# matthiasverstraete/3d_recognizer

Measured on AMD Instinct MI355X. Metric: training clouds/sec, N=40960 pts, bs=8, at 1/2/4/8 GPUs; mIoU parity, higher is better.
Workload: dtype f32 storage/accumulate, bf16x3 MFMA in the wide GEMMs

## Files before the change

3d_recognizer_amd/csrc/knn_grid.hip:

```cpp
#include "rl_common.h"
#include <stdlib.h>

namespace {

constexpr int KNN_SB = 3;


struct GridGeom {
    float lo[3];
    float inv[3];
    float h[3];
    int n[3];
    int ncell;
    float slack;
};

__device__ __forceinline__ unsigned enc(float f) {
    const unsigned u = __float_as_uint(f);
    return (u & 0x80000000u) ? ~u : (u | 0x80000000u);
}
__device__ __forceinline__ float dec(unsigned u) {
    return __uint_as_float((u & 0x80000000u) ? (u & 0x7fffffffu) : ~u);
}

constexpr int KNN_MAX_TASKS = 8;

struct KTask {
    const float* S;
    long s_bs;
    const float* Q;
    long q_bs;
    int Ns, Nq, k, self_mode;
    int32_t* idx32;
    int64_t* idx64;
    float* d2;
    GridGeom* geom;
    unsigned* bbox;
    int* count;
    int* start;
    int* cursor;
    float4* sorted;
    int cstride, maxcells;
    float per_cell;
    int lanes;
};

struct KMulti {
    int ntasks, B;
    int xcd;
    KTask t[KNN_MAX_TASKS];
};

__device__ __forceinline__ void knn_deal(const KMulti& m, int& b, int& bx) {
    if (m.xcd) {
        const int lin = (int)blockIdx.x + (int)gridDim.x * b;
        b = lin % m.B;
        bx = lin / m.B;
    }
}

__device__ __forceinline__ int kmax_of(int k) { return k == 1 ? 1 : k <= 4 ? 4 : k <= 8 ? 8 : k <= 16 ? 16 : k <= 32 ? 32 : 64; }

__global__ __launch_bounds__(256) void grid_init_kernel(const KMulti m) {
    const int task = blockIdx.y / m.B, b = blockIdx.y % m.B;
    const KTask& T = m.t[task];
    const int i = blockIdx.x * 256 + threadIdx.x;
    if (i < 6) T.bbox[b * 6 + i] = (i < 3) ? 0xffffffffu : 0u;
    int* cnt = T.count + (size_t)b * T.cstride;
    for (int e = i; e < T.cstride; e += gridDim.x * 256) cnt[e] = 0;
}

__global__ __launch_bounds__(256) void grid_bbox_kernel(const KMulti m) {
    const int task = blockIdx.y / m.B, b = blockIdx.y % m.B;
    const KTask& T = m.t[task];
    if (blockIdx.x * 256 >= T.Ns) return;
    const float* Sb = T.S + (size_t)b * T.s_bs * 3;
    float mn[3] = {INFINITY, INFINITY, INFINITY}, mx[3] = {-INFINITY, -INFINITY, -INFINITY};
    for (int j = blockIdx.x * 256 + threadIdx.x; j < T.Ns; j += gridDim.x * 256) {
#pragma unroll
        for (int a = 0; a < 3; ++a) {
            const float v = Sb[(size_t)j * 3 + a];
            mn[a] = fminf(mn[a], v);
            mx[a] = fmaxf(mx[a], v);
        }
    }
#pragma unroll
    for (int a = 0; a < 3; ++a) {
#pragma unroll
        for (int o = 32; o > 0; o >>= 1) {
            mn[a] = fminf(mn[a], __shfl_xor(mn[a], o, 64));
            mx[a] = fmaxf(mx[a], __shfl_xor(mx[a], o, 64));
        }
    }
    __shared__ float red[4][6];
    if ((threadIdx.x & 63) == 0) {
#pragma unroll
        for (int a = 0; a < 3; ++a) {
// ... 138 lines not shown
    }
}

template <int KMAX, int SB>
__device__ __forceinline__ void take_batch(const float4 (&cand)[SB], unsigned valid, float qx, float qy, float qz,
                                           unsigned long long (&best)[KMAX]) {
    unsigned long long key[SB];
    unsigned pass = 0;
#pragma unroll
    for (int i = 0; i < SB; ++i) {
        const float4 c = cand[i];
        const float dx = __fsub_rn(qx, c.x), dy = __fsub_rn(qy, c.y), dz = __fsub_rn(qz, c.z);
        const float d = __fadd_rn(__fadd_rn(__fmul_rn(dx, dx), __fmul_rn(dy, dy)), __fmul_rn(dz, dz));
        key[i] = ((unsigned long long)__float_as_uint(d) << 32) | (unsigned)__float_as_int(c.w);
        if (((valid >> i) & 1u) && key[i] < best[KMAX - 1]) pass |= 1u << i;
    }
    while (pass) {
        const int i = __ffs(pass) - 1;
        pass &= pass - 1;
        unsigned long long kk = key[0];
#pragma unroll
        for (int j = 1; j < SB; ++j)
            if (j == i) kk = key[j];
        insert_key<KMAX>(kk, best);
    }
}

template <int KMAX>
__device__ __forceinline__ void scan_range(const float4* __restrict__ pts, int begin, int end, float qx, float qy,
                                           float qz, unsigned long long (&best)[KMAX]) {
    constexpr int SB = KNN_SB;
    for (int t = begin; t < end; t += SB) {
        float4 cand[SB];
        unsigned valid = 0;
#pragma unroll
        for (int i = 0; i < SB; ++i) {
            cand[i] = pts[min(t + i, end - 1)];
            if (t + i < end) valid |= 1u << i;
        }
        take_batch<KMAX, SB>(cand, valid, qx, qy, qz, best);
    }
}

__device__ __forceinline__ int centre_out(int t) { return (t & 1) ? -((t + 1) >> 1) : (t >> 1); }

__device__ __forceinline__ float axis_gap(const GridGeom& g, int a, int ci, float q) {
    const float lo = g.lo[a] + (float)ci * g.h[a];
    const float hi = lo + g.h[a];
    float gap = fmaxf(lo - q, q - hi);
    gap -= g.slack;
    return gap > 0.f ? gap : 0.f;
}

template <int KMAX>
__device__ __forceinline__ void query_one_lane(const KTask& T, int b, int bx) {
    const int k = T.k, Nq = T.Nq, Ns = T.Ns;
    const int t = bx * 256 + threadIdx.x;
    if (t >= Nq) return;
    const int self_mode = T.self_mode;
    const float* Q = T.Q;
    const long q_bs = T.q_bs;
    int32_t* idx32 = T.idx32;
    int64_t* idx64 = T.idx64;
    float* d2out = T.d2;
    const GridGeom g = T.geom[b];
    const float4* pts = T.sorted + (size_t)b * Ns;
    const int* st = T.start + (size_t)b * T.cstride;
    float qx, qy, qz;
    int qi;
    if (self_mode) {
        const float4 me = pts[t];
        qx = me.x; qy = me.y; qz = me.z;
        qi = __float_as_int(me.w);
    } else {
        const float* p = Q + ((size_t)b * q_bs + t) * 3;
        qx = p[0]; qy = p[1]; qz = p[2];
        qi = t;
    }
    int c[3];
    cell_coords(g, qx, qy, qz, c);
    unsigned long long best[KMAX];
#pragma unroll
    for (int s = 0; s < KMAX; ++s) best[s] = KEY_EMPTY;

    const float q3[3] = {qx, qy, qz};
    for (int r = 0;; ++r) {
        const int z0 = max(c[2] - r, 0), z1 = min(c[2] + r, g.n[2] - 1);
        const int y0 = max(c[1] - r, 0), y1 = min(c[1] + r, g.n[1] - 1);
        const int x0 = max(c[0] - r, 0), x1 = min(c[0] + r, g.n[0] - 1);
        for (int tz = 0; tz <= 2 * r; ++tz) {
            const int z = c[2] + centre_out(tz);
            if (z < z0 || z > z1) continue;
            const bool zedge = (z == c[2] - r) || (z == c[2] + r);
            const float dz = axis_gap(g, 2, z, qz);
            for (int ty = 0; ty <= 2 * r; ++ty) {
                const int y = c[1] + centre_out(ty);
                if (y < y0 || y > y1) continue;
                const bool full_row = zedge || y == c[1] - r || y == c[1] + r;
                const float dy = axis_gap(g, 1, y, qy);
                const float dyz = dy * dy + dz * dz;
                const int row = (z * g.n[1] + y) * g.n[0];
                unsigned long long kth = best[KMAX - 1];
                if (k != KMAX) {
#pragma unroll
                    for (int s = 0; s < KMAX; ++s)
                        if (s == k - 1) kth = best[s];
                }
                const bool have = kth != KEY_EMPTY;
                const float lim = have ? __uint_as_float((unsigned)(kth >> 32)) * 1.00001f + 1e-30f : INFINITY;
                if (dyz > lim) continue;
                if (full_row) {
                    int xa = x0, xb = x1;
                    while (xa <= xb) {
                        const float gx = axis_gap(g, 0, xa, qx);
                        if (gx * gx + dyz > lim) ++xa; else break;
                    }
                    while (xb >= xa) {
                        const float gx = axis_gap(g, 0, xb, qx);
                        if (gx * gx + dyz > lim) --xb; else break;
                    }
                    if (xa <= xb) scan_range<KMAX>(pts, st[row + xa], st[row + xb + 1], qx, qy, qz, best);
                } else {
#pragma unroll
                    for (int e = 0; e < 2; ++e) {
                        const int x = e == 0 ? c[0] - r : c[0] + r;
                        if (x < x0 || x > x1 || (e == 1 && r == 0)) continue;
                        const float dxg = axis_gap(g, 0, x, qx);
                        if (dxg * dxg + dyz > lim) continue;
                        scan_range<KMAX>(pts, st[row + x], st[row + x + 1], qx, qy, qz, best);
                    }
                }
            }
        }
        const bool covers = (c[0] - r <= 0) && (c[0] + r >= g.n[0] - 1) && (c[1] - r <= 0) && (c[1] + r >= g.n[1] - 1) &&
                            (c[2] - r <= 0) && (c[2] + r >= g.n[2] - 1);
        if (covers) break;
        unsigned long long kth = best[KMAX - 1];
#pragma unroll
        for (int s = 0; s < KMAX; ++s)
            if (s == k - 1) kth = best[s];
        if (kth != KEY_EMPTY) {
            float bound = INFINITY;
#pragma unroll
            for (int a = 0; a < 3; ++a) {
                if (c[a] - r > 0) bound = fminf(bound, q3[a] - (g.lo[a] + (float)(c[a] - r) * g.h[a]));
                if (c[a] + r < g.n[a] - 1) bound = fminf(bound, (g.lo[a] + (float)(c[a] + r + 1) * g.h[a]) - q3[a]);
            }
            bound -= g.slack;
            const float kd = __uint_as_float((unsigned)(kth >> 32));
            if (bound > 0.f && kd < bound * bound * 0.999999f) break;
        }
    }
    const size_t o = ((size_t)b * Nq + qi) * k;
#pragma unroll
    for (int s = 0; s < KMAX; ++s) {
        if (s < k) {
            const bool empty = best[s] == KEY_EMPTY;
            const unsigned id = empty ? 0xffffffffu : (unsigned)(best[s] & 0xffffffffull);
            if (idx32) idx32[o + s] = (int32_t)id;
            if (idx64) idx64[o + s] = (int64_t)id;
            d2out[o + s] = __uint_as_float(empty ? 0xffffffffu : (unsigned)(best[s] >> 32));
        }
    }
}

template <int LANES>
__device__ __forceinline__ unsigned long long group_min(unsigned long long v) {
#pragma unroll
    for (int o = 1; o < LANES; o <<= 1) {
        const unsigned lo = __shfl_xor((unsigned)v, o, 64), hi = __shfl_xor((unsigned)(v >> 32), o, 64);
        const unsigned long long w = ((unsigned long long)hi << 32) | lo;
        v = w < v ? w : v;
    }
    return v;
}
template <int LANES>
__device__ __forceinline__ unsigned long long group_max(unsigned long long v) {
#pragma unroll
    for (int o = 1; o < LANES; o <<= 1) {
        const unsigned lo = __shfl_xor((unsigned)v, o, 64), hi = __shfl_xor((unsigned)(v >> 32), o, 64);
        const unsigned long long w = ((unsigned long long)hi << 32) | lo;
        v = w > v ? w : v;
    }
    return v;
}

template <int KMAX, int LANES>
__device__ __forceinline__ unsigned long long group_bound(const unsigned long long (&best)[KMAX], int k) {
    const int q = (k + LANES - 1) / LANES - 1;
    unsigned long long own_k = best[KMAX - 1], own_q = best[0];
#pragma unroll
    for (int s = 0; s < KMAX; ++s) {
        if (s == k - 1) own_k = best[s];
        if (s == q) own_q = best[s];
    }
    const unsigned long long a = group_min<LANES>(own_k), b = group_max<LANES>(own_q);
    return a < b ? a : b;
}

template <int KMAX, int LANES>
__device__ __forceinline__ void scan_range_n(const float4* __restrict__ pts, int begin, int end, int sub, float qx, float qy,
                                            float qz, unsigned long long (&best)[KMAX]) {
    constexpr int SB = KNN_SB;
    for (int t = begin + sub; t < end; t += LANES * SB) {
        float4 cand[SB];
        unsigned valid = 0;
#pragma unroll
        for (int i = 0; i < SB; ++i) {
            cand[i] = pts[min(t + LANES * i, end - 1)];
            if (t + LANES * i < end) valid |= 1u << i;
        }
        take_batch<KMAX, SB>(cand, valid, qx, qy, qz, best);
    }
}

template <int KMAX, int LANES>
__device__ __forceinline__ void query_n_lanes(const KTask& T, int b, int bx, unsigned long long* lds) {
    constexpr int QPB = 256 / LANES;
    unsigned long long (*lists)[LANES][KMAX] = reinterpret_cast<unsigned long long (*)[LANES][KMAX]>(lds);
    const int k = T.k, Nq = T.Nq, Ns = T.Ns;
    const int qslot = threadIdx.x / LANES, sub = threadIdx.x % LANES;
    const int t = bx * QPB + qslot;
    if (bx * QPB >= Nq) return;
    const bool active = t < Nq;
    unsigned long long best[KMAX];
#pragma unroll
    for (int s = 0; s < KMAX; ++s) best[s] = KEY_EMPTY;
    int qi = 0;
    if (active) {
        const GridGeom g = T.geom[b];
        const float4* pts = T.sorted + (size_t)b * Ns;
        const int* st = T.start + (size_t)b * T.cstride;
        float qx, qy, qz;
        if (T.self_mode) {
            const float4 me = pts[t];
            qx = me.x; qy = me.y; qz = me.z;
            qi = __float_as_int(me.w);
        } else {
            const float* p = T.Q + ((size_t)b * T.q_bs + t) * 3;
            qx = p[0]; qy = p[1]; qz = p[2];
            qi = t;
        }
        int c[3];
        cell_coords(g, qx, qy, qz, c);
        const float q3[3] = {qx, qy, qz};
        for (int r = 0;; ++r) {
            const int z0 = max(c[2] - r, 0), z1 = min(c[2] + r, g.n[2] - 1);
            const int y0 = max(c[1] - r, 0), y1 = min(c[1] + r, g.n[1] - 1);
            const int x0 = max(c[0] - r, 0), x1 = min(c[0] + r, g.n[0] - 1);
            for (int tz = 0; tz <= 2 * r; ++tz) {
                const int z = c[2] + centre_out(tz);
                if (z < z0 || z > z1) continue;
                const bool zedge = (z == c[2] - r) || (z == c[2] + r);
                const float dz = axis_gap(g, 2, z, qz);
                for (int ty = 0; ty <= 2 * r; ++ty) {
                    const int y = c[1] + centre_out(ty);
                    if (y < y0 || y > y1) continue;
                    const bool full_row = zedge || y == c[1] - r || y == c[1] + r;
                    const float dy = axis_gap(g, 1, y, qy);
                    const float dyz = dy * dy + dz * dz;
                    const int row = (z * g.n[1] + y) * g.n[0];
                    const unsigned long long kth = group_bound<KMAX, LANES>(best, k);
                    const float lim = kth != KEY_EMPTY ? __uint_as_float((unsigned)(kth >> 32)) * 1.00001f + 1e-30f : INFINITY;
                    if (dyz > lim) continue;
                    if (full_row) {
                        int xa = x0, xb = x1;
                        while (xa <= xb) {
                            const float gx = axis_gap(g, 0, xa, qx);
                            if (gx * gx + dyz > lim) ++xa; else break;
                        }
                        while (xb >= xa) {
                            const float gx = axis_gap(g, 0, xb, qx);
                            if (gx * gx + dyz > lim) --xb; else break;
                        }
                        if (xa <= xb) scan_range_n<KMAX, LANES>(pts, st[row + xa], st[row + xb + 1], sub, qx, qy, qz, best);
                    } else {
#pragma unroll
                        for (int e = 0; e < 2; ++e) {
                            const int x = e == 0 ? c[0] - r : c[0] + r;
                            if (x < x0 || x > x1 || (e == 1 && r == 0)) continue;
                            const float dxg = axis_gap(g, 0, x, qx);
                            if (dxg * dxg + dyz > lim) continue;
                            scan_range_n<KMAX, LANES>(pts, st[row + x], st[row + x + 1], sub, qx, qy, qz, best);
                        }
                    }
                }
            }
            const bool covers = (c[0] - r <= 0) && (c[0] + r >= g.n[0] - 1) && (c[1] - r <= 0) && (c[1] + r >= g.n[1] - 1) &&
                                (c[2] - r <= 0) && (c[2] + r >= g.n[2] - 1);
            if (covers) break;
            const unsigned long long kth = group_bound<KMAX, LANES>(best, k);
            if (kth != KEY_EMPTY) {
                float bound = INFINITY;
#pragma unroll
                for (int a = 0; a < 3; ++a) {
                    if (c[a] - r > 0) bound = fminf(bound, q3[a] - (g.lo[a] + (float)(c[a] - r) * g.h[a]));
                    if (c[a] + r < g.n[a] - 1) bound = fminf(bound, (g.lo[a] + (float)(c[a] + r + 1) * g.h[a]) - q3[a]);
                }
                bound -= g.slack;
                const float kd = __uint_as_float((unsigned)(kth >> 32));
                if (bound > 0.f && kd < bound * bound * 0.999999f) break;
            }
        }
    }
#pragma unroll
    for (int s = 0; s < KMAX; ++s) lists[qslot][sub][s] = best[s];
    __syncthreads();
    if (active) {
        const size_t o = ((size_t)b * Nq + qi) * k;
#pragma unroll
        for (int s = 0; s < KMAX; ++s) {
            const unsigned long long key = best[s];
            if (key == KEY_EMPTY) continue;
            int rank = s;
#pragma unroll
            for (int j = 1; j < LANES; ++j) {
                const unsigned long long* L = lists[qslot][(sub + j) % LANES];
                int lo = 0;
#pragma unroll
                for (int w = KMAX / 2; w >= 1; w >>= 1)
                    if (L[lo + w - 1] < key) lo += w;
                if (lo < KMAX && L[lo] < key) ++lo;
                rank += lo;
            }
            if (rank < k) {
                const unsigned id = (unsigned)(key & 0xffffffffull);
                if (T.idx32) T.idx32[o + rank] = (int32_t)id;
                if (T.idx64) T.idx64[o + rank] = (int64_t)id;
                T.d2[o + rank] = __uint_as_float((unsigned)(key >> 32));
            }
        }
    }
}

template <int KMAX>
__global__ __launch_bounds__(256, KMAX <= 16 ? 4 : 1) void grid_query_kernel(const KMulti m) {
    __shared__ unsigned long long lds[KMAX <= 16 ? 256 * KMAX : 1];
    const int task = blockIdx.y / m.B;
    int b = blockIdx.y % m.B, bx = blockIdx.x;
    knn_deal(m, b, bx);
    const KTask& T = m.t[task];
    if (kmax_of(T.k) != KMAX) return;
    if constexpr (KMAX <= 16) {
        if (T.lanes == 4) { query_n_lanes<KMAX, 4>(T, b, bx, lds); return; }
        if (T.lanes == 2) { query_n_lanes<KMAX, 2>(T, b, bx, lds); return; }
    }
    query_one_lane<KMAX>(T, b, bx);
}

struct Plan {
    int maxcells, cstride;
    float per_cell;
    size_t off_geom, off_bbox, off_count, off_start, off_cursor, off_sorted, bytes;
};

Plan make_plan(int B, int Ns, int k) {
    Plan p;
    constexpr float occ = 0.5f;
    p.per_cell = fmaxf(2.f, occ * (float)k);
    const long want = (long)((double)Ns / p.per_cell) + 1;
    p.maxcells = (int)(4 * want + 64);
    p.cstride = p.maxcells + 1;
    size_t o = 0;
    auto take = [&](size_t n) { size_t at = o; o += (n + 255) & ~(size_t)255; return at; };
    p.off_geom = take(sizeof(GridGeom) * B);
    p.off_bbox = take(sizeof(unsigned) * 6 * B);
    p.off_count = take(sizeof(int) * (size_t)p.cstride * B);
    p.off_start = take(sizeof(int) * (size_t)p.cstride * B);
    p.off_cursor = take(sizeof(int) * (size_t)p.cstride * B);
    p.off_sorted = take(sizeof(float4) * (size_t)Ns * B);
    p.bytes = o;
    return p;
}

void bind(KTask* t, const Plan& p, char* w) {
    t->geom = (GridGeom*)(w + p.off_geom);
    t->bbox = (unsigned*)(w + p.off_bbox);
    t->count = (int*)(w + p.off_count);
    t->start = (int*)(w + p.off_start);
    t->cursor = (int*)(w + p.off_cursor);
    t->sorted = (float4*)(w + p.off_sorted);
    t->cstride = p.cstride;
    t->maxcells = p.maxcells;
    t->per_cell = p.per_cell;
}

inline int lanes_for(long queries, int k) {
    if (k > 16) return 1;
    return queries >= 16384 ? 1 : 4;
}

int run_multi(const KMulti& m_in, hipStream_t st) {
    KMulti m = m_in;
    m.xcd = (m.B > 1 && 8 % m.B == 0) ? 1 : 0;
    for (int i = 0; i < m.ntasks; ++i) m.t[i].lanes = lanes_for((long)m.B * m.t[i].Nq, m.t[i].k);
    int maxNs = 1, maxNq = 1, maxc = 1;
    bool need[6] = {false, false, false, false, false, false};
    for (int i = 0; i < m.ntasks; ++i) {
        maxNs = max(maxNs, m.t[i].Ns);
        maxNq = max(maxNq, m.t[i].Nq);
        maxc = max(maxc, m.t[i].cstride);
        const int k = m.t[i].k;
        need[k == 1 ? 0 : k <= 4 ? 1 : k <= 8 ? 2 : k <= 16 ? 3 : k <= 32 ? 4 : 5] = true;
    }
    const int clouds = m.ntasks * m.B;
    int gi = rl_cdiv(maxc, 256);
    if (gi > 64) gi = 64;
    hipLaunchKernelGGL(grid_init_kernel, dim3(gi, clouds), dim3(256), 0, st, m);
    int gb = rl_cdiv(maxNs, 2048);
    if (gb > 16) gb = 16;
    hipLaunchKernelGGL(grid_bbox_kernel, dim3(gb, clouds), dim3(256), 0, st, m);
    hipLaunchKernelGGL(grid_geom_kernel, dim3(rl_cdiv(clouds, 64)), dim3(64), 0, st, m);
    hipLaunchKernelGGL(grid_count_kernel, dim3(rl_cdiv(maxNs, 256), clouds), dim3(256), 0, st, m);
    hipLaunchKernelGGL(grid_scan_kernel, dim3(clouds), dim3(1024), 0, st, m);
    hipLaunchKernelGGL(grid_scatter_kernel, dim3(rl_cdiv(maxNs, 256), clouds), dim3(256), 0, st, m);
    int gxq = 1;
    for (int i = 0; i < m.ntasks; ++i) gxq = max(gxq, rl_cdiv((long)m.t[i].Nq * m.t[i].lanes, 256));
    dim3 grid(gxq, clouds);
    if (need[0]) hipLaunchKernelGGL((grid_query_kernel<1>), grid, dim3(256), 0, st, m);
    if (need[1]) hipLaunchKernelGGL((grid_query_kernel<4>), grid, dim3(256), 0, st, m);
    if (need[2]) hipLaunchKernelGGL((grid_query_kernel<8>), grid, dim3(256), 0, st, m);
    if (need[3]) hipLaunchKernelGGL((grid_query_kernel<16>), grid, dim3(256), 0, st, m);
    if (need[4]) hipLaunchKernelGGL((grid_query_kernel<32>), grid, dim3(256), 0, st, m);
    if (need[5]) hipLaunchKernelGGL((grid_query_kernel<64>), grid, dim3(256), 0, st, m);
    rl_note_kernel("grid_query_kernel");
    RL_LAUNCH_CHECK("rl_knn(grid)");
    return RL_OK;
}

}

int64_t rl_knn_grid_workspace_bytes(int B, int Ns, int k) { return (int64_t)make_plan(B, Ns, k).bytes; }

int rl_knn_grid_run(const float* S, long s_bs, const float* Q, long q_bs, int B, int Ns, int Nq, int k, int32_t* i32,
                    int64_t* i64, float* d2, void* workspace, int64_t workspace_bytes, hipStream_t st) {
    const Plan p = make_plan(B, Ns, k);
    RL_REQUIRE(workspace && workspace_bytes >= (int64_t)p.bytes, RL_ERR_ARGS, "rl_knn: workspace too small (%ld < %ld bytes)",
               (long)workspace_bytes, (long)p.bytes);
    RL_REQUIRE(((uintptr_t)workspace & 255) == 0, RL_ERR_ARGS, "rl_knn: workspace must be 256-byte aligned");
    KMulti m;
    m.ntasks = 1;
    m.B = B;
    KTask& t = m.t[0];
    t.S = S; t.s_bs = s_bs; t.Q = Q; t.q_bs = q_bs; t.Ns = Ns; t.Nq = Nq; t.k = k;
    t.self_mode = (S == Q && s_bs == q_bs && Ns == Nq) ? 1 : 0;
    t.idx32 = i32; t.idx64 = i64; t.d2 = d2;
    bind(&t, p, (char*)workspace);
    return run_multi(m, st);
}

extern "C" int64_t rl_knn_multi_workspace_bytes(const rl_knn_task* tasks, int ntasks, int B) {
    if (!tasks || ntasks <= 0 || B <= 0) return 0;
    int64_t total = 0;
    for (int i = 0; i < ntasks; ++i) total += (int64_t)make_plan(B, tasks[i].Ns, tasks[i].k).bytes;
    return total;
}

extern "C" int rl_knn_multi(const rl_knn_task* tasks, int ntasks, int B, void* workspace, int64_t workspace_bytes,
                            void* stream) {
    RL_REQUIRE(tasks && ntasks > 0 && ntasks <= KNN_MAX_TASKS && B > 0 && B * ntasks <= 65535, RL_ERR_ARGS,
               "rl_knn_multi: 1..%d tasks expected", KNN_MAX_TASKS);
    RL_REQUIRE(workspace && ((uintptr_t)workspace & 255) == 0, RL_ERR_ARGS, "rl_knn_multi: workspace must be 256-byte aligned");
    KMulti m;
    m.ntasks = ntasks;
    m.B = B;
    size_t off = 0;
    for (int i = 0; i < ntasks; ++i) {
        const rl_knn_task& u = tasks[i];
        RL_REQUIRE(u.support && u.query && u.idx_out && u.d2_out && u.Nq > 0 && u.k > 0, RL_ERR_ARGS, "rl_knn_multi: bad task %d", i);
        RL_REQUIRE(u.Ns >= u.k, RL_ERR_FEW_SUPPORT, "Not enough points in support to find %d neighboors", u.k);
        RL_REQUIRE(u.k <= RL_KNN_MAX_K, RL_ERR_UNSUPPORTED, "rl_knn_multi: k=%d exceeds RL_KNN_MAX_K=%d", u.k, RL_KNN_MAX_K);
        RL_REQUIRE(u.support_bstride >= u.Ns && u.query_bstride >= u.Nq, RL_ERR_ARGS, "rl_knn_multi: batch stride smaller than the cloud");
        const Plan p = make_plan(B, u.Ns, u.k);
        RL_REQUIRE((int64_t)(off + p.bytes) <= workspace_bytes, RL_ERR_ARGS, "rl_knn_multi: workspace too small");
        KTask& t = m.t[i];
        t.S = u.support; t.s_bs = u.support_bstride; t.Q = u.query; t.q_bs = u.query_bstride;
        t.Ns = u.Ns; t.Nq = u.Nq; t.k = u.k;
        t.self_mode = (u.support == u.query && u.support_bstride == u.query_bstride && u.Ns == u.Nq) ? 1 : 0;
        t.idx32 = u.idx_out; t.idx64 = nullptr; t.d2 = u.d2_out;
        bind(&t, p, (char*)workspace + off);
        off += p.bytes;
    }
    return run_multi(m, (hipStream_t)stream);
// ... 2 lines not shown
```

3d_recognizer_amd/randlanet/_hip.py:

```python
import ctypes as C
import os
from typing import Optional

import torch

_LIB: Optional[C.CDLL] = None
_LIB_PATH = os.path.join(os.path.dirname(os.path.dirname(os.path.abspath(__file__))), "csrc",
                         "librandla_hip.so")
_LIB_PATH = os.environ.get("RL_HIP_LIB", _LIB_PATH)

ABI_VERSION = 110
MAX_SLOTS = 1024
KNN_MAX_K = 64
ACT_NONE, ACT_RELU, ACT_LRELU = 0, 1, 2

ERR_ARGS, ERR_FEW_SUPPORT, ERR_LAUNCH, ERR_UNSUPPORTED = -1, -2, -3, -4


class HipKernelError(RuntimeError):
    pass


class GemmDesc(C.Structure):
    _fields_ = [
# ... 219 lines not shown
    "rl_wgrad_plan": (_i, [C.POINTER(WgradDesc), C.POINTER(C.c_int32), C.POINTER(C.c_int32), C.POINTER(C.c_char_p)]),
    "rl_wgrad_plan2": (_i, [C.POINTER(WgradDesc), C.POINTER(C.c_int32), C.POINTER(C.c_int32), C.POINTER(C.c_char_p),
                            C.POINTER(C.c_int32), C.POINTER(C.c_int64), C.POINTER(C.c_int32), C.POINTER(C.c_char_p)]),
    "rl_gemm_plan": (_i, [C.POINTER(GemmDesc), C.POINTER(C.c_int32), C.POINTER(C.c_int32), C.POINTER(C.c_int32), C.POINTER(C.c_int32),
                          C.POINTER(C.c_int32), C.POINTER(C.c_char_p), C.POINTER(C.c_char_p)]),
    "rl_wgrad_nsplit": (_i, [_l, _i, _i]),
    "rl_wgrad_batchable": (_i, [C.POINTER(WgradDesc)]),
    "rl_wgrad_batch": (_i, [C.POINTER(WgradDesc), _i, _vp]),
    "rl_wgrad_reduce_batch": (_i, [C.POINTER(WgradReduceItem), _i, _vp]),
    "rl_bn_finalize": (_i, [_vp, _i, _l, _i, _vp, _vp, _vp, _vp, _vp, _f, _f, _i, _vp, _vp, _vp, _vp, _vp, _i, _vp, _vp]),
    "rl_bn_finalize_batch": (_i, [C.POINTER(BnFinalizeItem), _i, _vp]),
    "rl_bn_bwd_finalize_batch": (_i, [C.POINTER(BnBwdFinalizeItem), _i, _vp]),
    "rl_head_supported": (_i, [_i, _i]),
    "rl_head_grid": (_i, [_l]),
    "rl_head_fwd": (_i, [C.POINTER(HeadDesc), _vp, _vp]),
    "rl_head_bwd": (_i, [C.POINTER(HeadDesc), _vp]),
    "rl_bn_bwd_finalize_pair": (_i, [_vp, _vp, _i, _l, _i, _vp, _vp, _vp, _vp, _vp, _vp, _vp]),
    "rl_bn_reduce_slots": (_i, [_vp, _i, _i, _vp, _vp]),
    "rl_bn_bwd_slots": (_i, [_l]),
    "rl_bn_bwd_reduce": (_i, [C.POINTER(BnBwdDesc), _vp]),
    "rl_bn_bwd_finalize": (_i, [_vp, _i, _l, _i, _vp, _vp, _vp, _vp]),
    "rl_bn_bwd_apply": (_i, [C.POINTER(BnBwdDesc), _vp]),
    "rl_bn_bwd_fused_supported": (_i, [_l, _i, _l]),
    "rl_bn_bwd_fused": (_i, [C.POINTER(BnBwdDesc), _l, _vp, _vp, _vp, _vp]),
    "rl_resid_bn_bwd_supported": (_i, [_l, _i]),
    "rl_resid_bn_bwd_reduce": (_i, [C.POINTER(ResidBnBwdDesc), _vp]),
    "rl_resid_bn_bwd_apply": (_i, [C.POINTER(ResidBnBwdDesc), _vp]),
    "rl_resid_bn_bwd_fused_supported": (_i, [_l, _i]),
    "rl_resid_bn_bwd_fused": (_i, [C.POINTER(ResidBnBwdDesc), _vp, _vp, _vp, _vp, _vp]),
    "rl_copy_rows": (_i, [C.POINTER(RowsDesc), _vp]),
    "rl_copy_rows_pair": (_i, [C.POINTER(RowsDesc), C.POINTER(RowsDesc), _vp]),
    "rl_scatter_add_rows": (_i, [C.POINTER(RowsDesc), _vp]),
    "rl_csr_workspace_bytes": (_l, [C.POINTER(CsrTask), _i, _i]),
    "rl_csr_build": (_i, [C.POINTER(CsrTask), _i, _i, _vp, _l, _vp]),
    "rl_segment_sum_rows": (_i, [C.POINTER(SegsumDesc), _vp]),
    "rl_pool_supported": (_i, [_i, _i]),
    "rl_pool_slab_floats": (_l, [_l, _i]),
    "rl_pool_bwd_slots": (_i, [_l, _i]),
    "rl_pool_bwd_grid": (_i, [_l, _i, _i]),
    "rl_pool_fwd_slots": (_i, [_l, _i]),
    "rl_pool_fwd": (_i, [C.POINTER(PoolDesc), _vp]),
    "rl_rpe_stats_slots": (_i, [_l]),
    "rl_rpe_stats": (_i, [C.POINTER(PoolDesc), _vp, _vp]),
    "rl_rpe_bn_reduce": (_i, [C.POINTER(PoolDesc), _vp, _vp, _vp]),
    "rl_rpe_wgrad_slab_floats": (_l, [_l, _i, _i]),
    "rl_rpe_wgrad": (_i, [C.POINTER(PoolDesc), _vp, _vp, _vp, _l, _vp, _vp]),
    "rl_pool_bwd": (_i, [C.POINTER(PoolDesc), _vp]),
    "rl_set_pool128_x": (_i, [C.c_char_p]),
    "rl_get_pool128_x": (C.c_char_p, []),
    "rl_set_pool256_x": (_i, [C.c_char_p]),
    "rl_get_pool256_x": (C.c_char_p, []),
    "rl_set_decoder_cat": (_i, [C.c_char_p]),
    "rl_get_decoder_cat": (C.c_char_p, []),
    "rl_gemm_concat_supported": (_i, [C.POINTER(GemmDesc)]),
    "rl_attpool_cat_supported": (_i, [C.POINTER(AttpoolSrc), _l, _i, _i]),
    "rl_attpool_fwd_cat": (_i, [C.POINTER(AttpoolSrc), _vp, _l, _i, _i, _vp, _vp]),
    "rl_attpool_bwd_cat": (_i, [C.POINTER(AttpoolSrc), _vp, _vp, _vp, _l, _i, _i, _vp, _vp, _vp]),
    "rl_attpool_fwd": (_i, [_vp, _vp, _l, _i, _i, _vp, _vp]),
    "rl_attpool_bwd": (_i, [_vp, _vp, _vp, _vp, _l, _i, _i, _vp, _vp, _vp]),
    "rl_add_act_fwd": (_i, [_vp, _vp, _vp, _vp, _vp, _vp, _l, _i, _f, _vp, _vp]),
    "rl_add_act_bwd": (_i, [_vp, _vp, _l, _i, _f, _vp]),
    "rl_rpe_build": (_i, [_vp, _l, _vp, _vp, _i, _i, _i, _vp, _vp]),
    "rl_rpe_build_dist": (_i, [_vp, _l, _vp, _vp, _i, _i, _i, _vp, _vp]),
    "rl_batch_assemble": (_i, [_vp, _i, _i, _i, _vp, _vp, _vp, _vp, _vp, _vp]),
    "rl_batch_assemble_scratch_doubles": (_l, [_i, _i]),
    "rl_batch_assemble_flag_u32": (_l, [_i, _i, _i]),
    "rl_batch_draw": (_i, [_vp, _i, _i, C.c_uint64, _vp, _vp, _vp]),
    "rl_scale_mask": (_i, [_vp, _vp, _f, _l, _vp]),
    "rl_dropout_tick": (_i, [_vp, _vp, _vp]),
    "rl_dropout_fwd": (_i, [_vp, _vp, _vp, _i, _f, _vp, _l, _l, _i, _vp, C.c_uint64, _f, _vp]),
    "rl_dropout_bwd": (_i, [_vp, _l, _l, _i, _vp, C.c_uint64, _f, _vp]),
    "rl_upsample_cf": (_i, [_vp, _vp, _vp, _i, _i, _i, _i, _i, _i, _vp, _vp]),
    "rl_logits_unpermute": (_i, [_vp, _vp, _i, _i, _i, _vp, _vp]),
    "rl_logits_permute_grad": (_i, [_vp, _vp, _i, _i, _i, _vp, _vp]),
    "rl_logits_unpermute_b": (_i, [_vp, _vp, C.c_int64, _i, _i, _i, _vp, _vp]),
    "rl_logits_permute_grad_b": (_i, [_vp, _vp, C.c_int64, _i, _i, _i, _vp, _vp]),
    "rl_band_sort_workspace_bytes": (C.c_int64, [_i, _i, _vp, _i]),
    "rl_band_sort": (_i, [_vp, C.c_int64, _vp, _i, _i, _vp, _i, _vp, _vp, C.c_int64, _vp]),
    "rl_loss_max_classes": (_i, []),
    "rl_loss_work_doubles": (_l, [_l, _i]),
    "rl_loss_forward": (_i, [_vp, _vp, _i, _i, _i, _i, _f, _f, _i, _vp, _vp, _vp]),
    "rl_loss_backward": (_i, [_vp, _vp, _i, _i, _i, _i, _f, _f, _i, _vp, _f, _vp, _vp]),
    "rl_loss_forward_masked": (_i, [_vp, _vp, _i, _i, _i, _i, _f, _f, _i, _vp, _i, _vp, _vp, _vp]),
    "rl_loss_backward_masked": (_i, [_vp, _vp, _i, _i, _i, _i, _f, _f, _i, _vp, _f, _vp, _i, _vp, _vp]),
    "rl_loss_partials": (_i, [_vp, _vp, _i, _i, _i, _i, _f, _vp, _vp]),
    "rl_loss_totals_offset": (_l, [_i]),
    "rl_loss_from_totals": (_i, [_l, _i, _i, _f, _f, _i, _vp, _vp, _vp]),
    "rl_loss_backward_global": (_i, [_vp, _vp, _i, _i, _i, _i, _f, _f, _i, _vp, _f, _l, _vp, _vp]),
    "rl_lovasz_workspace_bytes": (_l, [_i, _i, _i]),
    "rl_lovasz_coef_offset": (_l, [_i, _i, _i]),
    "rl_lovasz_forward": (_i, [_vp, _vp, _i, _i, _i, _i, _vp, _vp, _l, _vp, _vp]),
    "rl_lovasz_backward": (_i, [_vp, _vp, _i, _i, _i, _i, _vp, _vp, _l, _f, _vp, _vp]),
    "rl_softmax_cf": (_i, [_vp, _i, _i, _i, _vp, _vp]),
    "rl_adam_step": (_i, [_vp, _vp, _vp, _vp, _l, _vp, _f, _f, _f, _f, _vp, _vp]),
    "rl_scene_workspace_bytes": (_l, [_l, _i]),
    "rl_scene_crop": (_i, [_vp, _l, _i, _vp, _i, _vp, _l, _vp, _vp, _l, _vp]),
    "rl_scene_accumulate": (_i, [_vp, _i, _i, _vp, _f, _f, _vp, _vp, _l, _vp]),
    "rl_scene_min_count": (_i, [_vp, _l, _vp, _vp, _vp]),
    "rl_scene_crop_padded": (_i, [_vp, _l, _i, _vp, _i, _vp, _l, _vp, _vp, _l, _vp]),
    "rl_scene_accumulate_first": (_i, [_vp, _i, _i, _vp, _f, _f, _vp, _vp, _l, _l, _i, _vp]),
    "rl_scenes_workspace_bytes": (_l, [_i, _l, _i]),
    "rl_scenes_init": (_i, [_vp, _i, _l, _vp, _vp, _l, _vp]),
    "rl_scenes_crop": (_i, [_vp, _i, _i, _l, _vp, _i, _i, _vp, _vp, _vp, _vp, _l, _vp]),
    "rl_scenes_crop_padded": (_i, [_vp, _i, _i, _l, _vp, _i, _i, _vp, _vp, _vp, _vp, _l, _vp]),
    "rl_scenes_vote_crop": (_i, [_vp, _i, _i, _l, _vp, _vp, _vp, _i, _i, _i, _i, _vp, _l, _l, _vp, _vp, _vp, _vp, _vp, _l, _vp]),
    "rl_scenes_vote_accumulate": (_i, [_vp, _i, _i, _l, _l, _i, _vp, _vp, _f, _f, _vp, _l, _vp]),
# ... 115 lines not shown
```

3d_recognizer_amd/randlanet/_ops.py:

```python
import contextlib
import ctypes as C
import os
from dataclasses import dataclass
from typing import Optional, Tuple

import torch

from . import _hip as H

F32 = torch.float32
BF16 = torch.bfloat16

_STORAGE = os.environ.get("RL_STORAGE", "f32")


def set_storage(mode: str) -> None:
    global _STORAGE
    if mode not in ("f32", "bf16"):
        raise ValueError(f"storage must be 'f32' or 'bf16', got {mode!r}")
    if mode == "bf16" and get_wide_gemm() == "fp32":
        raise H.HipKernelError("bf16 storage needs the bf16x3 / bf16 arithmetic mode (RL_WIDE_GEMM)")
    _STORAGE = mode


# ... 259 lines not shown
    def u(self) -> Lazy:
        return self.skip

    @property
    def g(self) -> Lazy:
        return self.x

    @property
    def idx(self) -> torch.Tensor:
        return self.nn

    @property
    def B(self) -> int:
        return self.skip.B

    @property
    def n(self) -> int:
        return self.skip.n

    @property
    def C(self) -> int:
        return self.x.C + self.skip.C

    @property
    def rows(self) -> int:
        return self.skip.rows


_CONCAT = (ConcatGather, InterpConcat)


def set_pool128_x(mode: str) -> None:
    H.check(H.lib().rl_set_pool128_x(mode.encode()), "rl_set_pool128_x")


def get_pool128_x() -> str:
    return H.lib().rl_get_pool128_x().decode()


def set_pool256_x(mode: str) -> None:
    H.check(H.lib().rl_set_pool256_x(mode.encode()), "rl_set_pool256_x")


def get_pool256_x() -> str:
    return H.lib().rl_get_pool256_x().decode()


def set_decoder_cat(mode: str) -> None:
    H.check(H.lib().rl_set_decoder_cat(mode.encode()), "rl_set_decoder_cat")


def get_decoder_cat() -> str:
    return H.lib().rl_get_decoder_cat().decode()


def _fill_a(d, a):
    if isinstance(a, _CONCAT):
        u, g, idx = a.u, a.g, a.idx
        _dev_check(g.raw, g.scale, g.shift, idx)
        assert idx.dtype == torch.int32 and idx.numel() == u.rows and u.bstride == u.n and g.B == u.B
        assert g.raw.dtype == F32 and g.raw.dim() == 2 and g.raw.shape[1] >= g.C
        assert g.raw.shape[0] >= (g.B - 1) * g.bstride + g.n, "second source rows out of range"
        M, _ = _fill_a(d, u)
        d.K = u.C + g.C
        d.a2_split, d.A2, d.lda2, d.a2_bstride, d.a2_idx = u.C, g.raw.data_ptr(), g.raw.shape[1], g.bstride, idx.data_ptr()
        if a.first:
            d.a2_split, d.a2_first = g.C, 1
        if g.scale is not None:
            assert g.scale.numel() == g.C and g.shift.numel() == g.C
            d.a2_scale, d.a2_shift, d.a2_act, d.a2_slope = g.scale.data_ptr(), g.shift.data_ptr(), g.act, g.slope
        return M, u.C + g.C
    if isinstance(a, Rpe):
        _dev_check(a.xyz, a.idx, a.d2)
        assert a.idx.dtype == torch.int32 and a.idx.shape == (a.B, a.n, a.K) and a.d2.shape == a.idx.shape
        assert a.xyz.shape[0] == a.B and a.xyz.shape[1] >= a.n and a.xyz.shape[2] == 3
        d.a_mode = 1
        d.xyz, d.xyz_bstride = a.xyz.data_ptr(), a.xyz.shape[1]
        d.nbr_idx, d.nbr_d2, d.nbr_k = a.idx.data_ptr(), a.d2.data_ptr(), a.K
        d.B, d.n, d.K = a.B, a.n, 10
        return a.rows, 10
    _dev_check(a.raw, a.scale, a.shift)
    assert a.raw.dtype in (F32, BF16) and a.raw.dim() == 2 and a.raw.shape[1] >= a.C
    assert a.raw.shape[0] >= (a.B - 1) * a.bstride + a.n, "A operand rows out of range"
    d.a_mode = 0
    d.A, d.lda, d.a_bstride = a.raw.data_ptr(), a.raw.shape[1], a.bstride
    if a.scale is not None:
        assert a.scale.numel() == a.C and a.shift.numel() == a.C
        d.in_scale, d.in_shift, d.in_act, d.in_slope = a.scale.data_ptr(), a.shift.data_ptr(), a.act, a.slope
    d.B, d.n, d.K = a.B, a.n, a.C
    return a.rows, a.C


def weight_strides(W: torch.Tensor, transposed: bool, K: int, N: int) -> Tuple[int, int]:
    if transposed:
        assert W.shape[0] == K and W.shape[1] == N, (tuple(W.shape), K, N)
        return N, 1
    assert W.shape[0] == N and W.shape[1] == K, (tuple(W.shape), K, N)
    return 1, K




def split_weights(entries) -> dict:
    out_map = {}
    if get_wide_gemm() == "fp32" or not entries:
        return out_map
# ... 1651 lines not shown
```

include/rl_randlanet.h:

```cpp
#ifndef RL_RANDLANET_H
#define RL_RANDLANET_H

#include <stdint.h>

#ifdef __cplusplus
extern "C" {
#endif

#define RL_VERSION 110

#define RL_OK 0
#define RL_ERR_ARGS (-1)
#define RL_ERR_FEW_SUPPORT (-2)
#define RL_ERR_LAUNCH (-3)
#define RL_ERR_UNSUPPORTED (-4)

#define RL_MAX_SLOTS 1024
#define RL_KNN_MAX_K 64
#define RL_MAX_CLASSES 256

const char* rl_last_error(void);
const char* rl_last_kernel(void);
int rl_version(void);
int64_t rl_launch_count(void);
int rl_spin_us(int us, void* stream);

int rl_row_blocks(int64_t rows, int rows_per_tile);

int64_t rl_knn_workspace_bytes(int B, int Ns, int Nq, int k);
int rl_knn_f32(const float* support, const float* query, int B, int Ns, int Nq, int k,
               int64_t* idx_out, float* d2_out, void* workspace, int64_t workspace_bytes,
               void* stream);

int rl_knn_f32_cpu(const float* support, const float* query, int B, int Ns, int Nq, int k,
                   int64_t* idx_out, float* d2_out);

int rl_knn_i32(const float* support, int64_t support_bstride, const float* query,
               int64_t query_bstride, int B, int Ns, int Nq, int k, int32_t* idx_out,
               float* d2_out, void* workspace, int64_t workspace_bytes, void* stream);

typedef struct rl_knn_task {
    const float* support;
    int64_t support_bstride;
    const float* query;
    int64_t query_bstride;
    int32_t Ns, Nq, k;
    int32_t* idx_out;
    float* d2_out;
} rl_knn_task;

int64_t rl_knn_multi_workspace_bytes(const rl_knn_task* tasks, int ntasks, int B);
int rl_knn_multi(const rl_knn_task* tasks, int ntasks, int B, void* workspace, int64_t workspace_bytes,
                 void* stream);

typedef struct rl_gemm_desc {
    const float* A;
    int64_t lda, a_bstride;
    int32_t a_mode;
    int32_t in_act;
    float in_slope;
    const float* in_scale;
    const float* in_shift;
    const float* xyz;
    int64_t xyz_bstride;
    const int32_t* nbr_idx;
    const float* nbr_d2;
    int32_t nbr_k;
    int32_t B, n, N, K;
    const float* W;
    int64_t w_ks, w_ns;
    const float* bias;
    float* Y;
    int64_t ldy, y_bstride;
    int32_t accumulate;
    double* stats;
    float* kslab;
    int64_t kslab_floats;
    const float* addend;
    float* out2;
    const int32_t* out2_index;
    int64_t out2_bstride;
    int32_t split_col;
    const void* W_split;
    const float* stats_pivot_mean;
    const float* stats_pivot_bias;
    const float* bnb_Y;
    const float* bnb_scale;
    const float* bnb_shift;
    const float* bnb_mean;
    const float* bnb_invstd;
    int32_t bnb_act;
    float bnb_slope;
    int32_t a2_split;
    int32_t a2_act;
    const float* A2;
    int64_t lda2, a2_bstride;
    const int32_t* a2_idx;
    const float* a2_scale;
    const float* a2_shift;
    float a2_slope;
    int32_t a2_first;
} rl_gemm_desc;

int rl_gemm_streams(const rl_gemm_desc* d);
int rl_gemm_concat_supported(const rl_gemm_desc* d);
int rl_gemm_plan(const rl_gemm_desc* d, int32_t* grid_xyz, int32_t* threads, int32_t* tile_bm_bn, int32_t* ksplit,
// ... 537 lines not shown
```

Before: 1321.

## Derive 1-NN upsampling indices from partner self-kNN search, fallback for misses

When a k=1 kNN task (query cloud onto a subsampled support that is a prefix of the same points) has a matching self-mode k>1 task on the same cloud, the k=1 answer is taken from the partner's neighbour list. It is the nearest neighbour whose index falls below the support size. Only queries where no such neighbour appears go through a separate miss kernel, which reuses the partner's grid when one matches. This drops a full grid build and a full k=1 query pass, at the cost of extra stores in the partner kernel, a miss-check launch, and a reliance on the support being a prefix of the partner's points.

```diff
diff --git a/3d_recognizer_amd/csrc/knn_grid.hip b/3d_recognizer_amd/csrc/knn_grid.hip
--- a/3d_recognizer_amd/csrc/knn_grid.hip
+++ b/3d_recognizer_amd/csrc/knn_grid.hip
@@ -1,5 +1,6 @@
 #include "rl_common.h"
 #include <stdlib.h>
+#include <string.h>
 
 namespace {
 
@@ -43,6 +44,10 @@
     int cstride, maxcells;
     float per_cell;
     int lanes;
+    int der_Ns;
+    int32_t* der_idx32;
+    int64_t* der_idx64;
+    float* der_d2;
 };
 
 struct KMulti {
@@ -287,11 +292,23 @@
     return gap > 0.f ? gap : 0.f;
 }
 
-template <int KMAX>
+__device__ __forceinline__ void store_derived(const KTask& T, size_t row, unsigned long long hit) {
+    const bool miss = hit == KEY_EMPTY;
+    const unsigned id = miss ? 0xffffffffu : (unsigned)(hit & 0xffffffffull);
+    if (T.der_idx32) T.der_idx32[row] = (int32_t)id;
+    if (T.der_idx64) T.der_idx64[row] = miss ? (int64_t)-1 : (int64_t)id;
+    T.der_d2[row] = __uint_as_float(miss ? 0xffffffffu : (unsigned)(hit >> 32));
+}
+__device__ __forceinline__ bool row_missing(const KTask& T, size_t row) {
+    return T.idx32 ? T.idx32[row] == -1 : T.idx64[row] == -1;
+}
+
+template <int KMAX, bool MISS>
 __device__ __forceinline__ void query_one_lane(const KTask& T, int b, int bx) {
     const int k = T.k, Nq = T.Nq, Ns = T.Ns;
     const int t = bx * 256 + threadIdx.x;
     if (t >= Nq) return;
+    if (MISS && !row_missing(T, (size_t)b * Nq + t)) return;
     const int self_mode = T.self_mode;
     const float* Q = T.Q;
     const long q_bs = T.q_bs;
@@ -397,6 +414,13 @@
             d2out[o + s] = __uint_as_float(empty ? 0xffffffffu : (unsigned)(best[s] >> 32));
         }
     }
+    if (!MISS && T.der_Ns) {
+        unsigned long long hit = KEY_EMPTY;
+#pragma unroll
+        for (int s = KMAX - 1; s >= 0; --s)
+            if (s < k && best[s] != KEY_EMPTY && (unsigned)(best[s] & 0xffffffffull) < (unsigned)T.der_Ns) hit = best[s];
+        store_derived(T, (size_t)b * Nq + qi, hit);
+    }
 }
 
 template <int LANES>
@@ -449,7 +473,7 @@
     }
 }
 
-template <int KMAX, int LANES>
+template <int KMAX, int LANES, bool MISS>
 __device__ __forceinline__ void query_n_lanes(const KTask& T, int b, int bx, unsigned long long* lds) {
     constexpr int QPB = 256 / LANES;
     unsigned long long (*lists)[LANES][KMAX] = reinterpret_cast<unsigned long long (*)[LANES][KMAX]>(lds);
@@ -457,7 +481,8 @@
     const int qslot = threadIdx.x / LANES, sub = threadIdx.x % LANES;
     const int t = bx * QPB + qslot;
     if (bx * QPB >= Nq) return;
-    const bool active = t < Nq;
+    bool active = t < Nq;
+    if (MISS && active) active = row_missing(T, (size_t)b * Nq + t);
     unsigned long long best[KMAX];
 #pragma unroll
     for (int s = 0; s < KMAX; ++s) best[s] = KEY_EMPTY;
@@ -543,6 +568,7 @@
     __syncthreads();
     if (active) {
         const size_t o = ((size_t)b * Nq + qi) * k;
+        unsigned long long hit = KEY_EMPTY;
 #pragma unroll
         for (int s = 0; s < KMAX; ++s) {
             const unsigned long long key = best[s];
@@ -563,7 +589,12 @@
                 if (T.idx32) T.idx32[o + rank] = (int32_t)id;
                 if (T.idx64) T.idx64[o + rank] = (int64_t)id;
                 T.d2[o + rank] = __uint_as_float((unsigned)(key >> 32));
+                if (!MISS && id < (unsigned)T.der_Ns && key < hit) hit = key;
             }
+        }
+        if (!MISS && T.der_Ns) {
+            hit = group_min<LANES>(hit);
+            if (sub == 0) store_derived(T, (size_t)b * Nq + qi, hit);
         }
     }
 }
@@ -577,10 +608,20 @@
     const KTask& T = m.t[task];
     if (kmax_of(T.k) != KMAX) return;
     if constexpr (KMAX <= 16) {
-        if (T.lanes == 4) { query_n_lanes<KMAX, 4>(T, b, bx, lds); return; }
-        if (T.lanes == 2) { query_n_lanes<KMAX, 2>(T, b, bx, lds); return; }
-    }
-    query_one_lane<KMAX>(T, b, bx);
+        if (T.lanes == 4) { query_n_lanes<KMAX, 4, false>(T, b, bx, lds); return; }
+        if (T.lanes == 2) { query_n_lanes<KMAX, 2, false>(T, b, bx, lds); return; }
+    }
+    query_one_lane<KMAX, false>(T, b, bx);
+}
+
+__global__ __launch_bounds__(256, 4) void grid_query_miss_kernel(const KMulti m) {
+    __shared__ unsigned long long lds[256];
+    const int task = blockIdx.y / m.B;
+    int b = blockIdx.y % m.B, bx = blockIdx.x;
+    knn_deal(m, b, bx);
+    const KTask& T = m.t[task];
+    if (T.lanes == 4) { query_n_lanes<1, 4, true>(T, b, bx, lds); return; }
+    query_one_lane<1, true>(T, b, bx);
 }
 
 struct Plan {
@@ -625,45 +666,109 @@
     return queries >= 16384 ? 1 : 4;
 }
 
+int g_knn_nn_derived = 1;
+
 int run_multi(const KMulti& m_in, hipStream_t st) {
-    KMulti m = m_in;
-    m.xcd = (m.B > 1 && 8 % m.B == 0) ? 1 : 0;
-    for (int i = 0; i < m.ntasks; ++i) m.t[i].lanes = lanes_for((long)m.B * m.t[i].Nq, m.t[i].k);
-    int maxNs = 1, maxNq = 1, maxc = 1;
+    KMulti search = m_in, build, miss;
+    const int B = m_in.B, nt = m_in.ntasks;
+    const int xcd = (B > 1 && 8 % B == 0) ? 1 : 0;
+    search.xcd = xcd;
+    for (int i = 0; i < nt; ++i) {
+        search.t[i].lanes = lanes_for((long)B * search.t[i].Nq, search.t[i].k);
+        search.t[i].der_Ns = 0;
+        search.t[i].der_idx32 = nullptr;
+        search.t[i].der_idx64 = nullptr;
+        search.t[i].der_d2 = nullptr;
+    }
+    int partner[KNN_MAX_TASKS];
+    bool own_grid[KNN_MAX_TASKS];
+    miss.ntasks = 0;
+    for (int i = 0; i < nt; ++i) {
+        partner[i] = -1;
+        own_grid[i] = true;
+        const KTask& T = search.t[i];
+        if (!g_knn_nn_derived || T.k != 1 || T.Ns > T.Nq) continue;
+        for (int j = 0; j < nt && partner[i] < 0; ++j) {
+            const KTask& P = search.t[j];
+            if (j != i && P.self_mode && P.k > 1 && !P.der_Ns && P.Q == T.Q && P.q_bs == T.q_bs && P.Nq == T.Nq && P.S == T.S &&
+                P.s_bs == T.s_bs)
+                partner[i] = j;
+        }
+        if (partner[i] < 0) continue;
+        KTask& P = search.t[partner[i]];
+        P.der_Ns = T.Ns;
+        P.der_idx32 = T.idx32;
+        P.der_idx64 = T.idx64;
+        P.der_d2 = T.d2;
+        KTask& M = miss.t[miss.ntasks++];
+        M = T;
+        M.self_mode = 0;
+        for (int j = 0; j < nt && own_grid[i]; ++j) {
+            const KTask& G = m_in.t[j];
+            if (j == i || !G.self_mode || G.k == 1 || G.S != T.S || G.s_bs != T.s_bs || G.Ns != T.Ns) continue;
+            M.geom = G.geom; M.start = G.start; M.sorted = G.sorted; M.cstride = G.cstride;
+            own_grid[i] = false;
+        }
+    }
+    build.B = miss.B = B;
+    build.xcd = miss.xcd = xcd;
+    build.ntasks = 0;
+    int ns = 0;
+    for (int i = 0; i < nt; ++i) {
+        if (own_grid[i]) build.t[build.ntasks++] = search.t[i];
+        if (partner[i] < 0) search.t[ns++] = search.t[i];
+    }
+    search.ntasks = ns;
+
+    int maxNs = 1, maxc = 1;
+    for (int i = 0; i < build.ntasks; ++i) {
+        maxNs = max(maxNs, build.t[i].Ns);
+        maxc = max(maxc, build.t[i].cstride);
+    }
     bool need[6] = {false, false, false, false, false, false};
-    for (int i = 0; i < m.ntasks; ++i) {
-        maxNs = max(maxNs, m.t[i].Ns);
-        maxNq = max(maxNq, m.t[i].Nq);
-        maxc = max(maxc, m.t[i].cstride);
-        const int k = m.t[i].k;
+    int gxq = 1;
+    for (int i = 0; i < search.ntasks; ++i) {
+        const int k = search.t[i].k;
         need[k == 1 ? 0 : k <= 4 ? 1 : k <= 8 ? 2 : k <= 16 ? 3 : k <= 32 ? 4 : 5] = true;
-    }
-    const int clouds = m.ntasks * m.B;
+        gxq = max(gxq, rl_cdiv((long)search.t[i].Nq * search.t[i].lanes, 256));
+    }
+    const int clouds = build.ntasks * B;
     int gi = rl_cdiv(maxc, 256);
     if (gi > 64) gi = 64;
-    hipLaunchKernelGGL(grid_init_kernel, dim3(gi, clouds), dim3(256), 0, st, m);
+    hipLaunchKernelGGL(grid_init_kernel, dim3(gi, clouds), dim3(256), 0, st, build);
     int gb = rl_cdiv(maxNs, 2048);
     if (gb > 16) gb = 16;
-    hipLaunchKernelGGL(grid_bbox_kernel, dim3(gb, clouds), dim3(256), 0, st, m);
-    hipLaunchKernelGGL(grid_geom_kernel, dim3(rl_cdiv(clouds, 64)), dim3(64), 0, st, m);
-    hipLaunchKernelGGL(grid_count_kernel, dim3(rl_cdiv(maxNs, 256), clouds), dim3(256), 0, st, m);
-    hipLaunchKernelGGL(grid_scan_kernel, dim3(clouds), dim3(1024), 0, st, m);
-    hipLaunchKernelGGL(grid_scatter_kernel, dim3(rl_cdiv(maxNs, 256), clouds), dim3(256), 0, st, m);
-    int gxq = 1;
-    for (int i = 0; i < m.ntasks; ++i) gxq = max(gxq, rl_cdiv((long)m.t[i].Nq * m.t[i].lanes, 256));
-    dim3 grid(gxq, clouds);
-    if (need[0]) hipLaunchKernelGGL((grid_query_kernel<1>), grid, dim3(256), 0, st, m);
-    if (need[1]) hipLaunchKernelGGL((grid_query_kernel<4>), grid, dim3(256), 0, st, m);
-    if (need[2]) hipLaunchKernelGGL((grid_query_kernel<8>), grid, dim3(256), 0, st, m);
-    if (need[3]) hipLaunchKernelGGL((grid_query_kernel<16>), grid, dim3(256), 0, st, m);
-    if (need[4]) hipLaunchKernelGGL((grid_query_kernel<32>), grid, dim3(256), 0, st, m);
-    if (need[5]) hipLaunchKernelGGL((grid_query_kernel<64>), grid, dim3(256), 0, st, m);
+    hipLaunchKernelGGL(grid_bbox_kernel, dim3(gb, clouds), dim3(256), 0, st, build);
+    hipLaunchKernelGGL(grid_geom_kernel, dim3(rl_cdiv(clouds, 64)), dim3(64), 0, st, build);
+    hipLaunchKernelGGL(grid_count_kernel, dim3(rl_cdiv(maxNs, 256), clouds), dim3(256), 0, st, build);
+    hipLaunchKernelGGL(grid_scan_kernel, dim3(clouds), dim3(1024), 0, st, build);
+    hipLaunchKernelGGL(grid_scatter_kernel, dim3(rl_cdiv(maxNs, 256), clouds), dim3(256), 0, st, build);
+    dim3 grid(gxq, search.ntasks * B);
+    if (need[1]) hipLaunchKernelGGL((grid_query_kernel<4>), grid, dim3(256), 0, st, search);
+    if (need[2]) hipLaunchKernelGGL((grid_query_kernel<8>), grid, dim3(256), 0, st, search);
+    if (need[3]) hipLaunchKernelGGL((grid_query_kernel<16>), grid, dim3(256), 0, st, search);
+    if (need[4]) hipLaunchKernelGGL((grid_query_kernel<32>), grid, dim3(256), 0, st, search);
+    if (need[5]) hipLaunchKernelGGL((grid_query_kernel<64>), grid, dim3(256), 0, st, search);
+    if (need[0]) hipLaunchKernelGGL((grid_query_kernel<1>), grid, dim3(256), 0, st, search);
+    if (miss.ntasks) {
+        int gxm = 1;
+        for (int i = 0; i < miss.ntasks; ++i) gxm = max(gxm, rl_cdiv((long)miss.t[i].Nq * miss.t[i].lanes, 256));
+        hipLaunchKernelGGL(grid_query_miss_kernel, dim3(gxm, miss.ntasks * B), dim3(256), 0, st, miss);
+    }
     rl_note_kernel("grid_query_kernel");
     RL_LAUNCH_CHECK("rl_knn(grid)");
     return RL_OK;
 }
 
 }
+
+extern "C" int rl_set_knn_nn(const char* mode) {
+    const bool derived = mode && !strcmp(mode, "derived"), searched = mode && !strcmp(mode, "searched");
+    RL_REQUIRE(derived || searched, RL_ERR_ARGS, "rl_set_knn_nn: mode must be \"derived\" or \"searched\"");
+    g_knn_nn_derived = derived ? 1 : 0;
+    return RL_OK;
+}
+extern "C" const char* rl_get_knn_nn(void) { return g_knn_nn_derived ? "derived" : "searched"; }
 
 int64_t rl_knn_grid_workspace_bytes(int B, int Ns, int k) { return (int64_t)make_plan(B, Ns, k).bytes; }
 
diff --git a/3d_recognizer_amd/randlanet/_hip.py b/3d_recognizer_amd/randlanet/_hip.py
--- a/3d_recognizer_amd/randlanet/_hip.py
+++ b/3d_recognizer_amd/randlanet/_hip.py
@@ -295,6 +295,8 @@
     "rl_get_pool256_x": (C.c_char_p, []),
     "rl_set_decoder_cat": (_i, [C.c_char_p]),
     "rl_get_decoder_cat": (C.c_char_p, []),
+    "rl_set_knn_nn": (_i, [C.c_char_p]),
+    "rl_get_knn_nn": (C.c_char_p, []),
     "rl_gemm_concat_supported": (_i, [C.POINTER(GemmDesc)]),
     "rl_attpool_cat_supported": (_i, [C.POINTER(AttpoolSrc), _l, _i, _i]),
     "rl_attpool_fwd_cat": (_i, [C.POINTER(AttpoolSrc), _vp, _l, _i, _i, _vp, _vp]),
diff --git a/3d_recognizer_amd/randlanet/_ops.py b/3d_recognizer_amd/randlanet/_ops.py
--- a/3d_recognizer_amd/randlanet/_ops.py
+++ b/3d_recognizer_amd/randlanet/_ops.py
@@ -335,6 +335,14 @@
 
 def get_decoder_cat() -> str:
     return H.lib().rl_get_decoder_cat().decode()
+
+
+def set_knn_nn(mode: str) -> None:
+    H.check(H.lib().rl_set_knn_nn(mode.encode()), "rl_set_knn_nn")
+
+
+def get_knn_nn() -> str:
+    return H.lib().rl_get_knn_nn().decode()
 
 
 def _fill_a(d, a):
diff --git a/include/rl_randlanet.h b/include/rl_randlanet.h
--- a/include/rl_randlanet.h
+++ b/include/rl_randlanet.h
@@ -52,6 +52,8 @@
 int64_t rl_knn_multi_workspace_bytes(const rl_knn_task* tasks, int ntasks, int B);
 int rl_knn_multi(const rl_knn_task* tasks, int ntasks, int B, void* workspace, int64_t workspace_bytes,
                  void* stream);
+int rl_set_knn_nn(const char* mode);
+const char* rl_get_knn_nn(void);
 
 typedef struct rl_gemm_desc {
     const float* A;
```

Result: no change. 1327, median of 6 (+0.4%).
